# VainF/Diff-Pruning

Hardware: AMD Instinct MI355X
Metric: importance-scored images/sec (UNet fwd+bwd+|w*dL/dw|) (higher is better)
Workload: dtype f32

## Files before the change

__graft_entry__.py:

```python
import importlib
import os
import subprocess
import sys

ROOT = os.path.dirname(os.path.abspath(__file__))
PKG = os.path.join(ROOT, 'diff-pruning_amd')
SRCS = ['csrc/gemm.hip', 'csrc/norm.hip', 'csrc/elementwise.hip', 'csrc/importance.hip', 'csrc/optim.hip', 'csrc/ema.hip', 'csrc/transformer.hip', 'csrc/replay.hip', 'csrc/attention.hip', 'csrc/winograd.hip', 'csrc/winograd43.hip', 'csrc/winograd2d.hip', 'csrc/wgrad2d.hip', 'csrc/vq.hip', 'csrc/sampler.hip', 'csrc/ups9.hip', 'csrc/ldm_sampler.hip', 'csrc/evalmetrics.hip', 'csrc/prune_global.hip', 'csrc/stage.hip', 'csrc/dpm_solver.hip', 'csrc/unipc.hip', 'csrc/magnitude.hip']


def _compile(variant_flags, out_name):
    from concurrent.futures import ThreadPoolExecutor
    hipcc = '/opt/rocm/bin/hipcc' if os.path.exists('/opt/rocm/bin/hipcc') else 'hipcc'
    objdir = os.path.join(PKG, 'build', out_name)
    os.makedirs(objdir, exist_ok=True)
    common = [hipcc, '--offload-arch=gfx950', '-O3', '-std=c++17', '-fPIC', '-I' + os.path.join(ROOT, 'include')] + variant_flags
    objs = [os.path.join(objdir, os.path.basename(s_)[:-4] + '.o') for s_ in SRCS]

    def one(i):
        subprocess.check_call(common + ['-c', os.path.join(PKG, SRCS[i]), '-o', objs[i]], cwd=PKG)
    with ThreadPoolExecutor(max_workers=min(len(SRCS), os.cpu_count() or 4)) as ex:
        list(ex.map(one, range(len(SRCS))))
    subprocess.check_call([hipcc, '--offload-arch=gfx950', '-shared', '-fPIC', '-o', os.path.join(PKG, out_name)] + objs, cwd=PKG)


def build():
    _compile([], 'libdp_hip.so')
    _compile(['-DDP_IEEE_SIGMOID'], 'libdp_hip_ieee.so')
    if ROOT not in sys.path:
        sys.path.insert(0, ROOT)
    lib = importlib.import_module('diff-pruning_amd._lib')
    lib._lib = None
    handle = lib.load()
    assert handle.dp_version() >= 100
    importlib.import_module('oracle.unet_ref')
    importlib.import_module('oracle.diffusion_ref')
    importlib.import_module('oracle.pruning_ref')


def smoke():
    import time
    import torch
    t_start = time.time()
    for p in (ROOT, os.path.join(ROOT, 'tests'), os.path.join(ROOT, 'tests', 'golden')):
        if p not in sys.path:
            sys.path.insert(0, p)
    gc = importlib.import_module('diff-pruning_amd.synthetic')
    from oracle import unet_ref, diffusion_ref
    from helpers import oracle_prune_replay
    unet = importlib.import_module('diff-pruning_amd.unet')
    diffusion = importlib.import_module('diff-pruning_amd.diffusion')
    sweep = importlib.import_module('diff-pruning_amd.sweep')
    graph_mod = importlib.import_module('diff-pruning_amd.graph')
    ops = importlib.import_module('diff-pruning_amd.ops')
    assert torch.cuda.is_available(), 'smoke() needs cuda:0'
    cfg = gc.TINY_CFG
    clean = torch.from_numpy(gc.det_clean((2, 3, 16, 16), 1))
    noise = torch.from_numpy(gc.det_noise((2, 3, 16, 16), 2))

    shapes = unet_ref.param_shapes(cfg)
    P = {n: torch.from_numpy(gc.det_param(n, s, 5)).requires_grad_(True) for n, s in shapes.items()}
# ... 94 lines not shown
```

diff-pruning_amd/_lib.py:

```python
import ctypes as C
import os

_HERE = os.path.dirname(os.path.abspath(__file__))
LIB_PATH = os.environ.get('DP_HIP_LIB') or os.path.join(_HERE, 'libdp_hip.so')

c_float_p = C.c_void_p
LL = C.c_longlong


class ConvGeom(C.Structure):
    _fields_ = [(n, C.c_int) for n in ('Ho', 'Wo', 'Hs', 'Ws', 'Hv', 'Wv', 'kw', 'stride', 'sden', 'pad_t', 'pad_l',
                                       'ups', 'c_split', '_pad')] + [('x1_img_stride', LL), ('x2_img_stride', LL)]


class ConvGemmParams(C.Structure):
    _fields_ = [('A', C.c_void_p), ('a_bs', LL), ('lda', C.c_int), ('a_kc', C.c_int),
                ('X1', C.c_void_p), ('X2', C.c_void_p), ('x_bs', LL),
                ('a_bytes', C.c_uint), ('x1_bytes', C.c_uint), ('x2_bytes', C.c_uint), ('_pad0', C.c_uint),
                ('g', ConvGeom),
                ('M', C.c_int), ('C', C.c_int), ('NPIX', C.c_int), ('ntaps', C.c_int), ('batches', C.c_int),
                ('tile', C.c_int),
                ('out', C.c_void_p), ('o_img_stride', LL), ('o_bs', LL),
                ('alpha', C.c_float), ('post_scale', C.c_float),
                ('bias', C.c_void_p), ('tadd', C.c_void_p), ('tadd_stride', LL),
# ... 14 lines not shown
                ('alpha', C.c_float), ('merge', C.c_int), ('ocs', LL),
                ('o_tap_stride', LL), ('o_col_stride', C.c_int), ('xcd', C.c_int), ('col_bias', C.c_void_p)]


class AttentionParams(C.Structure):
    _fields_ = [('q', C.c_void_p), ('k', C.c_void_p), ('v', C.c_void_p), ('o', C.c_void_p),
                ('q_bs', LL), ('k_bs', LL), ('v_bs', LL), ('o_bs', LL),
                ('N', C.c_int), ('heads', C.c_int), ('d', C.c_int), ('dv', C.c_int), ('T', C.c_int), ('scale', C.c_float),
                ('variant', C.c_int), ('_pad', C.c_int)]


class Dropout(C.Structure):
    _fields_ = [('thr24', C.c_uint), ('scale', C.c_float), ('seed', C.c_ulonglong), ('site', C.c_uint), ('step', C.c_uint),
                ('n_off', LL), ('step_dev', C.c_void_p)]


class ScoreMember(C.Structure):
    _fields_ = [('w', C.c_void_p), ('g', C.c_void_p), ('R', C.c_int), ('C', C.c_int), ('T', C.c_int), ('dim', C.c_int),
                ('mode', C.c_int), ('blk0', C.c_int), ('full_off', LL), ('col_off', LL), ('idx_off', LL)]


class SliceItem(C.Structure):
    _fields_ = [('src', C.c_void_p), ('dst', C.c_void_p), ('R', C.c_int), ('C', C.c_int), ('T', C.c_int), ('dim', C.c_int),
                ('n_keep', C.c_int), ('blk0', C.c_int), ('nblk', C.c_int), ('_pad', C.c_int), ('keep_off', LL)]


class ScoreEntry(C.Structure):
    _fields_ = [('m', ScoreMember), ('score_off', LL), ('n0', C.c_int), ('_pad', C.c_int)]


class MagMember(C.Structure):
    _fields_ = [('w', C.c_void_p), ('R', C.c_int), ('C', C.c_int), ('T', C.c_int), ('dim', C.c_int), ('n0', C.c_int),
                ('blk0', C.c_int), ('fold', C.c_int), ('_pad', C.c_int), ('idx_off', LL), ('row_off', LL)]


class MagGroup(C.Structure):
    _fields_ = [('row_off', LL), ('score_off', LL), ('n0', C.c_int), ('members', C.c_int)]


class PackItem(C.Structure):
    _fields_ = [('W', C.c_void_p), ('dst', C.c_void_p), ('Co', C.c_int), ('Ci', C.c_int), ('taps', C.c_int), ('mode', C.c_int),
                ('ld', C.c_int), ('blk0', C.c_int), ('nblk', C.c_int), ('_pad', C.c_int)]


class Ups9Params(C.Structure):
    _fields_ = [('U', C.c_void_p), ('dy', C.c_void_p), ('dx', C.c_void_p), ('dy_img_stride', LL), ('dx_img_stride', LL),
                ('u_bytes', C.c_uint), ('dy_bytes', C.c_uint)] + [(n, C.c_int) for n in ('ldu', 'N', 'M', 'K', 'H', 'W',
                                                                                         'accumulate', 'tile')]


class Ups9FwdParams(C.Structure):
    _fields_ = [('U', C.c_void_p), ('x', C.c_void_p), ('bias', C.c_void_p), ('y', C.c_void_p), ('x_img_stride', LL), ('y_img_stride', LL),
                ('u_bytes', C.c_uint), ('x_bytes', C.c_uint)] + [(n, C.c_int) for n in ('ldu', 'N', 'M', 'K', 'H', 'W')]


class ColsumItem(C.Structure):
    _fields_ = [('src', C.c_void_p), ('dst', C.c_void_p), ('N', C.c_int), ('C', C.c_int), ('wstride', C.c_int),
                ('woff', C.c_int), ('accumulate', C.c_int), ('ld', C.c_int)]


class DpmSolverCoef(C.Structure):
    _fields_ = [(n, C.c_float) for n in ('sigma_s', 'alpha_s', 'kx', 'k0', 'k1', 'k2', 'ir0', 'ir1', 'q', 'iq')]


class UniPCCoef(C.Structure):
    _fields_ = [(n, C.c_float) for n in ('sigma_s', 'alpha_s', 'c_cx', 'c_c0', 'c_cB', 'c_rk1', 'c_rk2', 'c_rho1', 'c_rho2', 'c_rho_last',
                                         'p_cx', 'p_c0', 'p_cB', 'p_rk1', 'p_rk2', 'p_rho1', 'p_rho2')]


_vp, _i, _f, _ll = C.c_void_p, C.c_int, C.c_float, LL
_dr = C.POINTER(Dropout)

SIGNATURES = {
    'dp_conv_gemm': [C.POINTER(ConvGemmParams), _vp],
    'dp_conv_wino': [C.POINTER(ConvGemmParams), _vp],
    'dp_conv_wino_supported': [C.POINTER(ConvGemmParams)],
    'dp_conv_splitk_epilogue': [C.POINTER(ConvGemmParams), _vp],
    'dp_pack_weight_wino': [_vp, _i, _i, _i, _vp, _i, _vp],
    'dp_conv_wino2d': [C.POINTER(ConvGemmParams), _vp],
    'dp_conv_wino2d_supported': [C.POINTER(ConvGemmParams)],
    'dp_pack_weight_wino2d': [_vp, _i, _i, _i, _vp, _i, _vp],
    'dp_conv_wino43': [C.POINTER(ConvGemmParams), _vp],
    'dp_conv_wino43_supported': [C.POINTER(ConvGemmParams)],
    'dp_pack_weight_wino43': [_vp, _i, _i, _vp, _i, _vp],
    'dp_wgrad_wino': [C.POINTER(NtGemmParams), _vp],
    'dp_wgrad_wino2d': [C.POINTER(NtGemmParams), _vp],
    'dp_wgrad_wino2d_supported': [C.POINTER(NtGemmParams)],
    'dp_wgrad_wino_supported': [C.POINTER(NtGemmParams)],
    'dp_nt_gemm': [C.POINTER(NtGemmParams), _vp],
    'dp_splitk_reduce': [_vp, _ll, _i, _vp, _ll, _i, _vp],
    'dp_splitk_reduce_taps': [_vp, _ll, _i, _vp, _ll, _i, _i, _vp],
    'dp_pack_weight': [_vp, _i, _i, _i, _i, _vp, _i, _vp],
    'dp_pack_weight_batch': [C.POINTER(PackItem), _i, _vp],
    'dp_groupnorm_silu_fwd': [_vp, _vp, _i, _ll, _ll, _vp, _vp, _i, _i, _i, _i, _f, _i, _vp, _ll, _vp, _dr, _vp],
    'dp_groupnorm_silu_bwd': [_vp, _vp, _i, _ll, _ll, _vp, _vp, _vp, _vp, _ll, _i, _i, _i, _i, _i, _vp, _ll, _vp, _ll,
                              _vp, _ll, _vp, _dr, _vp, _vp],
    'dp_groupnorm_silu_fwd_split': [_vp, _vp, _i, _ll, _ll, _vp, _vp, _i, _i, _i, _i, _f, _i, _vp, _ll, _vp, _i, _vp, _dr,
                                    _vp],
    'dp_groupnorm_silu_bwd_split': [_vp, _vp, _i, _ll, _ll, _vp, _vp, _vp, _vp, _ll, _i, _i, _i, _i, _i, _vp, _ll, _vp, _ll,
                                    _vp, _ll, _vp, _i, _vp, _dr, _vp],
    'dp_colsum_accum': [_vp, _i, _i, _i, _i, _vp, _i, _vp],
    'dp_colsum_accum_batch': [C.POINTER(ColsumItem), _i, _vp],
    'dp_rowsum_nc': [_vp, _ll, _i, _i, _i, _vp, _vp],
    'dp_silu_fwd': [_vp, _vp, _ll, _vp],
    'dp_silu_bwd': [_vp, _vp, _vp, _ll, _i, _vp],
    'dp_axpby': [_vp, _f, _vp, _f, _ll, _vp],
    'dp_copy_strided': [_vp, _ll, _vp, _ll, _i, _ll, _i, _vp],
    'dp_attention_fwd': [C.POINTER(AttentionParams), _vp],
    'dp_attention_fwd_supported': [_i, _i, _i],
    'dp_softmax_fwd': [_vp, _vp, _ll, _i, _vp],
    'dp_softmax_bwd': [_vp, _vp, _vp, _ll, _i, _f, _vp],
    'dp_timestep_embedding': [_vp, _i, _i, _i, _f, _f, _vp, _vp],
    'dp_add_noise': [_vp, _vp, _vp, _vp, _i, _ll, _vp, _vp],
    'dp_mse_fwd_bwd': [_vp, _vp, _ll, _f, _vp, _vp, _i, _vp, _vp],
    'dp_kd_fwd_bwd': [_vp, _vp, _vp, _ll, _f, _f, _f, _vp, _vp, _i, _vp],
    'dp_kd_terms': [_vp, _i, _f, _f, _f, _vp, _vp],
    'dp_early_exit_update': [_vp, _f, _vp, _vp, _i, _vp],
    'dp_zero_if_stopped': [_vp, _ll, _vp, _vp],
    'dp_early_exit_update_ratio': [_vp, _f, _vp, _vp, _i, _vp],
    'dp_randn_philox': [_vp, _ll, _ll, C.c_ulonglong, C.c_uint, C.c_uint, _vp],
    'dp_sum_partials': [_vp, _i, _f, _vp, _vp],
    'dp_downsum2x2': [_vp, _ll, _i, _i, _i, _i, _vp, _ll, _vp],
    'dp_upsample2x': [_vp, _ll, _i, _i, _i, _i, _vp, _ll, _vp],
    'dp_interleave2x2': [_vp, _ll, _ll, _i, _i, _i, _i, _vp, _ll, _vp, _ll, _vp],
    'dp_deinterleave2x2': [_vp, _ll, _i, _i, _i, _i, _vp, _ll, _ll, _vp],
    'dp_ups_weff': [_vp, _ll, _vp, _vp],
    'dp_ups_wfold': [_vp, _ll, _vp, _i, _vp],
    'dp_ups9_u': [_vp, _ll, _vp, _vp],
    'dp_ups9_dgrad': [C.POINTER(Ups9Params), _vp],
    'dp_ups9_dgrad_supported': [C.POINTER(Ups9Params)],
    'dp_ups9_fwd': [C.POINTER(Ups9FwdParams), _vp],
    'dp_wg_reduce': [_vp, _vp, _i, _i, _i, _i, _i, _vp, _i, _vp, _vp],
    'dp_gather_add': [_vp, _vp, _i, _vp, _vp],
    'dp_group_score': [C.POINTER(ScoreMember), _i, _i, _vp, _vp, _vp, _vp],
    'dp_slice_batch': [C.POINTER(SliceItem), _i, _vp, _vp],
    'dp_score_groups': [C.POINTER(ScoreEntry), _i, _vp, _vp, _ll, _vp, _ll, _vp, _ll, _vp],
    'dp_select_smallest_workspace': [_ll, _i],
    'dp_select_smallest': [_vp, _ll, C.POINTER(LL), _i, _ll, _vp, _ll, _vp, _vp, _vp],
    'dp_magnitude_max_width': [],
    'dp_magnitude_rows': [C.POINTER(MagMember), _i, _vp, _vp, _ll, _f, _i, _vp, _ll, _vp],
    'dp_magnitude_finish': [C.POINTER(MagGroup), _i, _vp, _vp, _ll, _i, _i, _i, _vp, _ll, _vp],
    'dp_sumsq_partials': [_vp, _ll, _vp, _i, _vp],
    'dp_clip_coef': [_vp, _i, _f, _vp, _vp, _vp],
    'dp_adam_ema': [_vp, _vp, _vp, _vp, _vp, _ll, _vp, _f, _f, _f, _f, _f, _f, _f, _vp],
    'dp_set_step_scalars': [_vp, _f, _f, _f, C.c_uint, _vp],
    'dp_adamw_ema': [_vp, _vp, _vp, _vp, _vp, _ll, _vp, _f, _f, _f, _f, _f, _f, _f, _f, _vp],
    'dp_embedding_bwd': [_vp, _vp, _i, _i, _vp, _vp],
    'dp_ema_update': [_vp, _vp, _ll, _f, _vp],
    'dp_fold_sum': [_vp, C.POINTER(C.c_void_p), _i, _ll, _vp],
    'dp_adam_ema_dev': [_vp, _vp, _vp, _vp, _vp, _ll, _vp, _vp, _f, _f, _f, _f, _vp],
    'dp_ddim_step': [_vp, _vp, _vp, _f, _f, _f, _i, _f, _vp, _ll, _vp],
    'dp_ddpm_step': [_vp, _vp, _vp, _f, _f, _f, _f, _f, _i, _f, _vp, _ll, _vp],
    'dp_denoise_step': [_vp, _vp, _vp, _i, _f, _f, _f, _f, _f, _f, _vp, _vp, _ll, _vp],
    'dp_image_to_u8': [_vp, _ll, _i, _i, _i, _i, _i, _vp, _vp],
    'dp_cfg_denoise_step': [_vp, _vp, _vp, _f, _i, _vp, _vp, _vp, _f, _f, _f, _f, _f, _f, _vp, _vp, _vp, _vp, _ll, _vp],
    'dp_dpm_solver_step': [_vp, _vp, _vp, _vp, _i, _i, C.POINTER(DpmSolverCoef), _vp, _vp, _ll, _vp],
    'dp_unipc_step': [_vp, _vp, _vp, _vp, _vp, _vp, _i, _i, _i, C.POINTER(UniPCCoef), _vp, _vp, _vp, _ll, _vp],
    'dp_dropout_apply': [_vp, _ll, _vp, _ll, _i, _ll, _dr, _vp],
    'dp_dropout_mask': [_vp, _ll, _ll, _dr, _vp],
    'dp_layernorm_fwd': [_vp, _ll, _vp, _vp, _i, _i, _i, _f, _vp, _ll, _vp, _vp],
    'dp_layernorm_bwd': [_vp, _ll, _vp, _vp, _vp, _ll, _i, _i, _i, _vp, _ll, _vp, _ll, _vp, _vp],
    'dp_geglu_fwd': [_vp, _i, _ll, _vp, _vp],
    'dp_geglu_bwd': [_vp, _vp, _i, _ll, _vp, _vp],
    'dp_add_rowvec': [_vp, _ll, _vp, _i, _i, _i, _vp, _ll, _vp],
    'dp_q_sample': [_vp, _vp, _vp, _vp, _vp, _i, _ll, _vp, _vp],
    'dp_cfg_combine': [_vp, _vp, _f, _vp, _ll, _vp],
    'dp_u8_to_float': [_vp, _i, _i, _i, _i, _i, _vp, _ll, _i, C.c_uint, _i, _dr, _vp],
    'dp_pool2d': [_vp, _ll, _i, _i, _i, _i, _i, _i, _i, _i, _vp, _ll, _vp],
    'dp_resize_bilinear': [_vp, _ll, _i, _i, _i, _i, _i, _i, _f, _f, _vp, _vp],
    'dp_ssim': [_vp, _vp, _i, _i, _i, _i, _f, _vp, _vp, _vp],
    'dp_ssim_workspace': [_i, _i, _i, _i],
    'dp_mse_per_image': [_vp, _vp, _i, _ll, _vp, _vp],
    'dp_em_row_norms2': [_vp, _ll, _i, _ll, _vp, _vp],
    'dp_em_knn_merge': [_vp, _ll, _ll, _ll, _vp, _vp, _i, _i, _vp, _vp],
    'dp_em_inside_ball': [_vp, _ll, _ll, _ll, _vp, _vp, _vp, _vp, _vp],
    'dp_em_poly_sums': [_vp, _i, _ll, _ll, _ll, _ll, C.c_double, C.c_double, _i, _vp, _i, _vp, _vp],
    'dp_em_isc_rows': [_vp, _ll, _i, _ll, _vp, _vp, _vp],
    'dp_em_isc_colmeans': [_vp, _ll, _vp, _ll, _ll, _i, _vp, _vp],
    'dp_vq_blocks': [_ll],
    'dp_vq_quantize': [_vp, _ll, _i, _i, _ll, _vp, _i, _vp, _ll, _vp, _vp, _vp],
    'dp_vq_loss': [_vp, _i, C.c_double, _vp, _vp],
    'dp_replay_build': [_vp, C.POINTER(C.c_void_p)],
    'dp_replay_launch': [_vp, _vp, _vp],
    'dp_replay_info': [_vp, C.POINTER(C.c_int)],
# ... 35 lines not shown
```

diff-pruning_amd/engine.py:

```python
import os

import torch

from . import ops

_SPEC3 = ops.ConvSpec(3, 1, 1, 0)
_SPEC1 = ops.ConvSpec(1, 1, 0, 0)
_SPEC_UP = ops.ConvSpec(3, 1, 1, 1)
UPS_COPY = not os.environ.get('DP_NO_UPS_COPY')
UPS_SUBPIXEL = not os.environ.get('DP_NO_UPS_SUBPIXEL')
_UPS_SPECS = ops.UPS_CLASS_SPECS
S2_PARITY = not os.environ.get('DP_NO_S2_PARITY')
FUSE_QKV_WGRAD = not os.environ.get('DP_NO_FUSED_QKV_WGRAD')
OVERLAP_MIN_WORK = 4_000_000

RES_DIFFUSERS = dict(norm1='.norm1', conv1='.conv1', temb='.time_emb_proj', norm2='.norm2', conv2='.conv2',
                     shortcut='.conv_shortcut', dropout='.dropout')
RES_LDM = dict(norm1='.in_layers.0', conv1='.in_layers.2', temb='.emb_layers.1', norm2='.out_layers.0',
               conv2='.out_layers.3', shortcut='.skip_connection')


SIDE_KEEP_MAX_BYTES = int(float(os.environ.get('DP_SIDE_KEEP_GB', '4')) * (1 << 30))


# ... 375 lines not shown
                  alpha=1.0, dx_add=None):
        w = self.P[name + '.weight']

        if rows is None and (name + '.bias') in self.P and self._rows_src is not None and self._rows_src[0].data_ptr() == dy.data_ptr():
            rows = self._rows_of(dy)

        def param_grads(rows):
            ops.conv_wgrad(dy, x, x2, self.G[name + '.weight'], spec, alpha=alpha, accumulate=True)
            if (name + '.bias') in self.P:
                if rows is None:
                    rows = ops.rowsum_nc(dy)
                if alpha != 1.0:
                    rows = rows.contiguous()
                    rows = ops.axpby(rows, alpha, torch.empty_like(rows), 0.0)
                self._colsum(rows, rows.shape[0], rows.shape[1], 1, 0, self.G[name + '.bias'])

        side = self._side_stream(dy, x, x2, rows)
        if side is None:
            param_grads(rows)
        else:
            with torch.cuda.stream(side):
                param_grads(rows)
        if not need_dx:
            return None
        if (S2_PARITY and spec.stride == 2 and spec.k == 3 and not spec.ups and spec.pad in (0, 1) and alpha == 1.0
                and dx_out is None and in_hw[0] == 2 * dy.shape[2] and in_hw[1] == 2 * dy.shape[3]):
            packs = [self.packs.get(name, w, ('s2', ph, pw, spec.pad)) for ph in (0, 1) for pw in (0, 1)]
            return ops.conv_dgrad_s2(dy, packs, w.shape[1], spec, in_hw, add=dx_add)
        wd, ldd = self.packs.get(name, w, 1)
        wino = None
        if w.dim() == 4 and w.shape[2] == 3 and hasattr(ops, 'wino_wanted') and tuple(in_hw) == tuple(dy.shape[2:]):
            wino = self._wino_operand(name, w, 1, w.shape[1], (w.shape[0],), dy.shape[0], dy.shape[2], dy.shape[3], spec)
        dx = ops.conv_dgrad(dy, wd, ldd, w.shape[1], spec, in_hw, alpha=alpha, out=dx_out, accumulate=dx_accumulate,
                            **({'wino': wino} if wino is not None else {}))
        if dx_add is not None:
            ops.copy_strided(dx_add, dx, accumulate=True)
        return dx

    def _ups_conv_fwd(self, name, x):
        w = self.P[name + '.weight']
        N, _, H, W = x.shape
        if hasattr(ops, 'ups9_fwd_wanted') and ops.ups9_fwd_wanted(N, w.shape[1], w.shape[0], H, W):
            up, ldu = self.packs.get(name, w, ('up9', 0, 0))
            return ops.ups9_fwd(x, up, ldu, w.shape[0], bias=self.P.get(name + '.bias'))
        q = ops.empty_act((4, N, w.shape[0], H, W), x.device)
        for c, spec in enumerate(_UPS_SPECS):
            wp, ld = self.packs.get(name, w, ('up', c, 0))
            ops.conv_forward(x, None, wp, ld, w.shape[0], spec, bias=self.P.get(name + '.bias'), out=q[c])
        return ops.interleave2x2(q)

    def _ups_conv_bwd(self, name, dy, x):
        w = self.P[name + '.weight']
        use9 = hasattr(ops, 'ups9_dgrad_wanted') and ops.ups9_dgrad_wanted(x.shape[0], w.shape[1], w.shape[0], x.shape[2], x.shape[3])
        dyq = None if use9 else ops.deinterleave2x2(dy)
        rows = None
        if (name + '.bias') in self.P and self._rows_src is not None and self._rows_src[0].data_ptr() == dy.data_ptr():
            rows = self._rows_of(dy)

        def param_grads(rows, dyq=dyq):
            if dyq is None:
                dyq = ops.deinterleave2x2(dy)
            gweff = torch.empty((4,) + tuple(w.shape[:2]) + (2, 2), dtype=torch.float32, device=dy.device)
            for c, spec in enumerate(_UPS_SPECS):
                ops.conv_wgrad(dyq[c], x, None, gweff[c], spec, accumulate=False)
            ops.ups_wfold(gweff, self.G[name + '.weight'], accumulate=True)
            if (name + '.bias') in self.P:
                if rows is None:
                    rows = ops.rowsum_nc(dy)
                self._colsum(rows, rows.shape[0], rows.shape[1], 1, 0, self.G[name + '.bias'])

        side = self._side_stream(dy, dyq, x, rows)
        if side is None:
            param_grads(rows)
        else:
            with torch.cuda.stream(side):
                param_grads(rows)
        if use9:
            up, ldu = self.packs.get(name, w, ('up9', 0, 1))
            return ops.ups9_dgrad(dy, up, ldu, w.shape[1])
        dx = None
        for c, spec in enumerate(_UPS_SPECS):
            wd, ldd = self.packs.get(name, w, ('up', c, 1))
            dx = ops.conv_dgrad(dyq[c], wd, ldd, w.shape[1], spec, tuple(x.shape[2:]), out=dx, accumulate=c > 0)
        return dx

    def _gn_param_grads(self, name, pws):
        N, C = pws.shape[0], pws.shape[1]
        self._colsum(pws, N, C, 2, 1, self.G[name + '.weight'])
        self._colsum(pws, N, C, 2, 0, self.G[name + '.bias'])

    def resnet_fwd(self, pre, xa, xb, semb, out_scale, save, names=RES_DIFFUSERS, G=None, eps=None):
        P, cfg = self.P, self.cfg
        G = cfg['norm_num_groups'] if G is None else G
        eps = cfg['norm_eps'] if eps is None else eps
        nm = names
        n1, st1 = ops.groupnorm_fwd(xa, xb, P[pre + nm['norm1'] + '.weight'], P[pre + nm['norm1'] + '.bias'], G, eps, True)
        if self._temb is not None:
            o, c = self._temb[1][pre]
            tproj = self._temb[2][:xa.shape[0], o:o + c]
        elif semb is None:
            tproj = None
        else:
            tproj = self._linear(pre + nm['temb'], semb)
        h = self._conv(pre + nm['conv1'], n1, None, _SPEC3, tadd=tproj)
        drop = self._drop(pre + nm['dropout']) if 'dropout' in nm else None
        n2, st2 = ops.groupnorm_fwd(h, None, P[pre + nm['norm2'] + '.weight'], P[pre + nm['norm2'] + '.bias'], G, eps, True,
                                    drop=drop)
        has_sc = (pre + nm['shortcut'] + '.weight') in P
        if has_sc:
            res = self._conv(pre + nm['shortcut'], xa, xb, _SPEC1)
        else:
            if xb is not None:
                res = torch.cat([xa, xb], 1)
            else:
                res = xa
        out = self._conv(pre + nm['conv2'], n2, None, _SPEC3, res=res, post_scale=1.0 / out_scale)
        if save is not None:
            save[pre] = (xa, xb, st1, n1, h, st2, n2, has_sc, out_scale, nm, G, drop)
# ... 315 lines not shown
```

diff-pruning_amd/ops.py:

```python
import ctypes as C
import os
import math
import torch

from . import _lib as L

_f32 = torch.float32


def _lib():
    return L.load()


_raw_stream = getattr(torch._C, '_cuda_getCurrentRawStream', None)


def _stream():
    if _raw_stream is not None:
        return C.c_void_p(_raw_stream(torch.cuda.current_device()))
    return C.c_void_p(torch.cuda.current_stream().cuda_stream)


def _p(t):
    return None if t is None else C.c_void_p(t.data_ptr())
# ... 709 lines not shown
    HW = H * W
    npix = HW * N
    if npix >= (1 << 29):
        return False
    if 9 * Cin * ldu * 4 != u_bytes or u_bytes >= _MAX_BYTES:
        return False
    if x_img_stride < HW * Cin or y_img_stride < 4 * HW * Cout or (y_img_stride & 1):
        return False
    if x_bytes < ((N - 1) * x_img_stride + HW * Cin) * 4 or x_bytes >= _MAX_BYTES:
        return False
    bm, bn = UPS9_FWD_TILE
    return -(-npix // bn) * -(-Cout // bm) < (1 << 31)


def ups9_fwd_gate(N, Cin, Cout, H, W):
    bm, bn = UPS9_FWD_TILE
    blocks = -(-(N * H * W) // bn) * -(-Cout // bm)
    return blocks >= UPS9_FWD_GATE_MIN_BLOCKS and max(Cin, Cout) <= UPS9_FWD_GATE_MAX_CH


def ups9_fwd_wanted(N, Cin, Cout, H, W):
    if not UPS9 or min(N, Cin, Cout, H, W) < 1 or N * H * W * max(Cin, 4 * Cout) * 4 >= _MAX_BYTES:
        return False
    return ups9_fwd_gate(N, Cin, Cout, H, W)


def _ups9_fwd_params(x, up, ldu, Cout, bias, out):
    sx, so = _chk_act(x), _chk_act(out)
    N, Cin, H, W = x.shape
    p = L.Ups9FwdParams()
    p.U, p.x, p.bias, p.y = _p(up), _p(x), _p(bias), _p(out)
    p.x_img_stride, p.y_img_stride = sx, so
    p.u_bytes, p.x_bytes = up.numel() * 4, _extent_bytes(x)
    p.ldu, p.N, p.M, p.K, p.H, p.W = ldu, N, Cout, Cin, H, W
    return p


def ups9_fwd(x, up, ldu, Cout, *, bias=None, out=None):
    N, Cin, H, W = x.shape
    if out is None:
        out = empty_act((N, Cout, 2 * H, 2 * W), x.device)
    assert out.shape == (N, Cout, 2 * H, 2 * W) and (bias is None or (bias.numel() == Cout and bias.is_contiguous()))
    p = _ups9_fwd_params(x, up, ldu, Cout, bias, out)
    ok = ups9_fwd_shape_ok(N, Cin, Cout, H, W, p.x_img_stride, p.y_img_stride, p.x_bytes, ldu, p.u_bytes, up.data_ptr(),
                           out.data_ptr(), bias.data_ptr() if bias is not None else 0)
    if not ok:
        raise ValueError('dp_ups9_fwd does not take this launch (ups9_fwd_shape_ok)')
    rc = _run(lambda: _lib().dp_ups9_fwd(C.byref(p), _stream()),
              _UPS9_FWD_NAME,
              2.0 * Cin * N * H * W * Cout * 9, 4.0 * (x.numel() + up.numel() + out.numel()))
    assert rc != 1, 'host shape rule and dp_ups9_fwd disagree (hipErrorInvalidValue for a launch ups9_fwd_shape_ok takes)'
    L.check(rc, 'dp_ups9_fwd')
    return out


_ws_cache = {}
WGRAD_BLOCKS = 1024
WGRAD_MIN_PIX = int(os.environ.get('DP_WGRAD_MIN_PIX', '128'))


def _workspace(n, device):
    if torch.cuda.is_current_stream_capturing():
        return torch.empty(max(n, 1), dtype=_f32, device=device)
    key = (device.index if device.index is not None else torch.cuda.current_device(), _stream().value)
    t = _ws_cache.get(key)
    if t is None or t.numel() < n:
        t = torch.empty(max(n, 1 << 22), dtype=_f32, device=device)
        _ws_cache[key] = t
    return t


WGRAD_WINO = os.environ.get('DP_WGRAD_WINO', '1') not in ('0', '')
WGRAD_WINO_MIN_FILL = float(os.environ.get('DP_WGRAD_WINO_MIN_FILL', '0.7'))
WGRAD_WINO_MIN_WORK = int(os.environ.get('DP_WGRAD_WINO_MIN_WORK', '512'))


WGRAD_WINO2D = os.environ.get('DP_WGRAD_WINO2D', '1') not in ('0', '')
WGRAD_WINO2D_BLOCKS = int(os.environ.get('DP_WGRAD_WINO2D_BLOCKS', '512'))
WGRAD_WINO2D_MIN_FILL = float(os.environ.get('DP_WGRAD_WINO2D_MIN_FILL', '0.7'))


def _nt_gemm_params(A, a_img_stride, x, x2, geom, M, Cc, ncols, ntaps, P, splits, pps, tile, alpha, ldo, batch=None):
    p = L.NtGemmParams()
    Z, a_bs, x_bs, batched = batch or (1, 0, 0, 0)
    p.A, p.a_bs, p.a_img_stride = _p(A), a_bs, a_img_stride
    p.X1, p.X2, p.x_bs = _p(x), _p(x2), x_bs
    if batch is None:
        p.a_bytes, p.x1_bytes, p.x2_bytes = _extent_bytes(A), _extent_bytes(x), _extent_bytes(x2)
    else:
        p.a_bytes, p.x1_bytes, p.x2_bytes = _checked_bytes(M * P * 4), _checked_bytes(ncols * P * 4), 0
    p.g = geom
    p.M, p.C, p.NCOLS, p.ntaps, p.P = M, Cc, ncols, ntaps, P
    p.batches, p.splits, p.p_per_split, p.tile, p.batched = Z, splits, pps, tile, batched
    p.alpha, p.ldo = alpha, ldo
    return p


def _wgrad_launch(p, gw, accumulate, sym, name, flops, label, taps, device):
    acc = 1 if accumulate else 0
    if p.splits == 1:
        p.out, p.o_bs, p.accumulate = _p(gw), 0, acc
        L.check(_run(lambda: getattr(_lib(), sym)(C.byref(p), _stream()), name, flops), label)
        return gw
    n = gw.numel()
    ws = _workspace(p.splits * n, device)
    p.out, p.o_bs, p.accumulate = _p(ws), n, 0
# ... 1069 lines not shown
```

include/dp_hip.h:

```cpp
#ifndef DP_HIP_H
#define DP_HIP_H
#include <stdint.h>
#ifdef __cplusplus
extern "C" {
#endif

typedef struct dp_conv_geom {
    int Ho, Wo, Hs, Ws, Hv, Wv, kw, stride, sden, pad_t, pad_l, ups, c_split, _pad;
    long long x1_img_stride, x2_img_stride;
} dp_conv_geom;

typedef struct dp_conv_gemm_params {
    const float* A; long long a_bs; int lda; int a_kc;
    const float* X1; const float* X2; long long x_bs;
    unsigned a_bytes, x1_bytes, x2_bytes, _pad0;
    dp_conv_geom g;
    int M, C, NPIX, ntaps, batches, tile;
    float* out; long long o_img_stride; long long o_bs;
    float alpha; float post_scale;
    const float* bias; const float* tadd; long long tadd_stride;
    const float* res; long long r_img_stride;
    int accumulate; int ksplit;
    float* ws;
    int x_guard; int act;
// ... 94 lines not shown
    long long q_bs, k_bs, v_bs, o_bs;
    int N, heads, d, dv, T;
    float scale;
    int variant;
    int _pad;
} dp_attention_params;
int dp_attention_fwd(const dp_attention_params* p, void* stream);
int dp_attention_fwd_supported(int T, int d, int dv);
int dp_softmax_bwd(const float* p, const float* dp, float* ds, long long rows, int cols, float scale, void* stream);

int dp_timestep_embedding(const float* t, int B, int dim, int flip_sin_to_cos, float freq_shift, float max_period, float* out, void* stream);

int dp_add_noise(const float* x0, const float* noise, const float* acp, const int64_t* t, int B, long long per_img, float* out, void* stream);

int dp_mse_fwd_bwd(const float* out, const float* noise, long long n, float gscale, float* dout, float* partial, int nblocks,
                   const float* stop_state, void* stream);
int dp_kd_fwd_bwd(const float* out, const float* teacher, const float* noise, long long n, float w_kd, float w_eps, float gscale,
                  float* dout, float* partial, int nblocks, void* stream);
int dp_kd_terms(const float* partial, int nblocks, float w_kd, float w_eps, float scale, float* terms, void* stream);
int dp_early_exit_update(const float* loss, float thr, float* state, float* losses, int max_steps, void* stream);
int dp_zero_if_stopped(float* x, long long n, const float* state, void* stream);
int dp_early_exit_update_ratio(const float* loss, float thr, float* state, float* losses, int max_steps, void* stream);
int dp_sum_partials(const float* partial, int n, float scale, float* dst, void* stream);

int dp_downsum2x2(const float* dy, long long dy_img_stride, int N, int C, int H, int W, float* dx, long long dx_img_stride, void* stream);

int dp_upsample2x(const float* x, long long x_img_stride, int N, int C, int H, int W, float* y, long long y_img_stride, void* stream);

int dp_interleave2x2(const float* q, long long q_class_stride, long long q_img_stride, int N, int C, int Ho, int Wo,
                     const float* add, long long add_img_stride, float* dx, long long dx_img_stride, void* stream);

int dp_deinterleave2x2(const float* y, long long y_img_stride, int N, int C, int Ho, int Wo, float* q,
                       long long q_class_stride, long long q_img_stride, void* stream);

int dp_ups_weff(const float* w, long long M, float* weff, void* stream);
int dp_ups_wfold(const float* gweff, long long M, float* gw, int accumulate, void* stream);

typedef struct dp_ups9_params {
    const float* U; const float* dy; float* dx;
    long long dy_img_stride, dx_img_stride;
    unsigned u_bytes, dy_bytes;
    int ldu, N, M, K, H, W, accumulate, tile;
} dp_ups9_params;
int dp_ups9_u(const float* w, long long M, float* u, void* stream);
int dp_ups9_dgrad(const dp_ups9_params* p, void* stream);
int dp_ups9_dgrad_supported(const dp_ups9_params* p);
typedef struct dp_ups9_fwd_params {
    const float* U; const float* x; const float* bias; float* y;
    long long x_img_stride, y_img_stride;
    unsigned u_bytes, x_bytes;
    int ldu, N, M, K, H, W;
} dp_ups9_fwd_params;
int dp_ups9_fwd(const dp_ups9_fwd_params* p, void* stream);

int dp_wg_reduce(const float* w, const float* g, int R, int C, int T, int dim, int mode, float* out, int accumulate,
                 float* scratch, void* stream);

int dp_gather_add(const float* src, const int64_t* idx, int n, float* dst, void* stream);

typedef struct dp_score_member {
    const float* w; const float* g;
    int R, C, T, dim, mode, blk0;
    long long full_off, col_off, idx_off;
} dp_score_member;
int dp_group_score(const dp_score_member* members, int n, int n0, const int64_t* idx, float* scratch, float* score, void* stream);
typedef struct dp_slice_item {
    const float* src; float* dst;
    int R, C, T, dim, n_keep, blk0, nblk, _pad;
    long long keep_off;
} dp_slice_item;
int dp_slice_batch(const dp_slice_item* items, int n, const int64_t* keep, void* stream);

typedef struct dp_score_entry {
    dp_score_member m;
    long long score_off;
    int n0, _pad;
} dp_score_entry;
int dp_score_groups(dp_score_entry* entries, int n, dp_score_entry* table_dev, const int64_t* idx, long long idx_len,
                    float* scratch, long long scratch_len, float* scores, long long n_scores, void* stream);
long long dp_select_smallest_workspace(long long n, int groups);
int dp_select_smallest(const float* scores, long long n, const long long* group_off, int groups, long long k, void* work,
                       long long work_bytes, int* out_dev, int* out_host, void* stream);

typedef struct dp_mag_member {
    const float* w;
    int R, C, T, dim, n0, blk0, fold, _pad;
    long long idx_off, row_off;
} dp_mag_member;
typedef struct dp_mag_group {
    long long row_off, score_off;
    int n0, members;
} dp_mag_group;
int dp_magnitude_max_width(void);
int dp_magnitude_rows(dp_mag_member* members, int n, dp_mag_member* table_dev, const int64_t* idx, long long idx_len,
                      float p, int root, float* rows, long long rows_len, void* stream);
int dp_magnitude_finish(const dp_mag_group* groups, int n, dp_mag_group* table_dev, const float* rows, long long rows_len,
                        int reduction, int normalizer, int lamp, float* scores, long long n_scores, void* stream);

int dp_sumsq_partials(const float* x, long long n, float* partial, int nblocks, void* stream);
int dp_set_step_scalars(float* hyper, float lr, float bc1, float bc2, unsigned step, void* stream);
int dp_adam_ema_dev(float* p, const float* g, float* m, float* v, float* ema, long long n, const float* clip_coef,
                    const float* hyper, float b1, float b2, float eps, float ema_decay, void* stream);
int dp_clip_coef(const float* partial, int n, float max_norm, float* norm_out, float* coef_out, void* stream);
int dp_adam_ema(float* p, const float* g, float* m, float* v, float* ema, long long n, const float* clip_coef,
                float lr, float b1, float b2, float eps, float bc1, float bc2, float ema_decay, void* stream);

// ... 106 lines not shown
```

Baseline: 5054.

## Add fused upsample-conv weight-gradient kernel with split-K MFMA and reduce

Adds a dedicated kernel for the weight gradient of the nearest-2x upsample followed by a 3x3 conv. It reads the interleaved dy directly and forms nine combined dy/x tap panels in shared memory, so one MFMA GEMM covers every tap. A split-K reduce kernel then folds the result back into 3x3 weights. This replaces deinterleaving dy, four separate conv_wgrad launches and the ups_wfold pass for large enough shapes. The trade-offs are a workspace of splits*9*Co*Ci floats and an extra reduce pass.

```diff
diff --git a/__graft_entry__.py b/__graft_entry__.py
--- a/__graft_entry__.py
+++ b/__graft_entry__.py
@@ -5,7 +5,7 @@
 
 ROOT = os.path.dirname(os.path.abspath(__file__))
 PKG = os.path.join(ROOT, 'diff-pruning_amd')
-SRCS = ['csrc/gemm.hip', 'csrc/norm.hip', 'csrc/elementwise.hip', 'csrc/importance.hip', 'csrc/optim.hip', 'csrc/ema.hip', 'csrc/transformer.hip', 'csrc/replay.hip', 'csrc/attention.hip', 'csrc/winograd.hip', 'csrc/winograd43.hip', 'csrc/winograd2d.hip', 'csrc/wgrad2d.hip', 'csrc/vq.hip', 'csrc/sampler.hip', 'csrc/ups9.hip', 'csrc/ldm_sampler.hip', 'csrc/evalmetrics.hip', 'csrc/prune_global.hip', 'csrc/stage.hip', 'csrc/dpm_solver.hip', 'csrc/unipc.hip', 'csrc/magnitude.hip']
+SRCS = ['csrc/gemm.hip', 'csrc/norm.hip', 'csrc/elementwise.hip', 'csrc/importance.hip', 'csrc/optim.hip', 'csrc/ema.hip', 'csrc/transformer.hip', 'csrc/replay.hip', 'csrc/attention.hip', 'csrc/winograd.hip', 'csrc/winograd43.hip', 'csrc/winograd2d.hip', 'csrc/wgrad2d.hip', 'csrc/vq.hip', 'csrc/sampler.hip', 'csrc/ups9.hip', 'csrc/ups9_wgrad.hip', 'csrc/ldm_sampler.hip', 'csrc/evalmetrics.hip', 'csrc/prune_global.hip', 'csrc/stage.hip', 'csrc/dpm_solver.hip', 'csrc/unipc.hip', 'csrc/magnitude.hip']
 
 
 def _compile(variant_flags, out_name):
diff --git a/diff-pruning_amd/_lib.py b/diff-pruning_amd/_lib.py
--- a/diff-pruning_amd/_lib.py
+++ b/diff-pruning_amd/_lib.py
@@ -90,6 +90,12 @@
 class Ups9FwdParams(C.Structure):
     _fields_ = [('U', C.c_void_p), ('x', C.c_void_p), ('bias', C.c_void_p), ('y', C.c_void_p), ('x_img_stride', LL), ('y_img_stride', LL),
                 ('u_bytes', C.c_uint), ('x_bytes', C.c_uint)] + [(n, C.c_int) for n in ('ldu', 'N', 'M', 'K', 'H', 'W')]
+
+
+class Ups9WgradParams(C.Structure):
+    _fields_ = [('dy', C.c_void_p), ('x', C.c_void_p), ('ws', C.c_void_p), ('gw', C.c_void_p), ('dy_img_stride', LL), ('x_img_stride', LL),
+                ('ws_floats', LL), ('dy_bytes', C.c_uint), ('x_bytes', C.c_uint)] + [(n, C.c_int) for n in (
+                    'N', 'Co', 'Ci', 'H', 'W', 'splits', 'tiles_per_split', 'ld', 'accumulate')]
 
 
 class ColsumItem(C.Structure):
@@ -168,6 +174,8 @@
     'dp_ups9_dgrad': [C.POINTER(Ups9Params), _vp],
     'dp_ups9_dgrad_supported': [C.POINTER(Ups9Params)],
     'dp_ups9_fwd': [C.POINTER(Ups9FwdParams), _vp],
+    'dp_ups9_wgrad': [C.POINTER(Ups9WgradParams), _vp],
+    'dp_ups9_wgrad_reduce': [C.POINTER(Ups9WgradParams), _vp],
     'dp_wg_reduce': [_vp, _vp, _i, _i, _i, _i, _i, _vp, _i, _vp, _vp],
     'dp_gather_add': [_vp, _vp, _i, _vp, _vp],
     'dp_group_score': [C.POINTER(ScoreMember), _i, _i, _vp, _vp, _vp, _vp],
diff --git a/diff-pruning_amd/csrc/ups9_wgrad.hip b/diff-pruning_amd/csrc/ups9_wgrad.hip
--- /dev/null
+++ b/diff-pruning_amd/csrc/ups9_wgrad.hip
@@ -0,0 +1,246 @@
+#include "dp_common.h"
+
+#define U9W_LAUNCH(k, ...) do { dp_launch_names[dp_launches++ & (DP_LAUNCH_RING - 1)] = #k; hipLaunchKernelGGL(k, __VA_ARGS__); } while (0)
+
+typedef float f32x2 __attribute__((ext_vector_type(2)));
+
+#define U9W_RSRC_FLAGS 0x00020000
+#define U9W_OOB 0x80000000u
+#define U9W_BM 64
+#define U9W_BN 64
+#define U9W_KP 16
+#define U9W_LD 66
+
+__device__ __forceinline__ __amdgpu_buffer_rsrc_t u9w_rsrc(const float* base, unsigned bytes) {
+    return __builtin_amdgcn_make_buffer_rsrc((void*)base, 0, (int)bytes, U9W_RSRC_FLAGS);
+}
+__device__ __forceinline__ float u9w_bload(__amdgpu_buffer_rsrc_t r, unsigned byte_off) {
+    asm volatile("" : "+v"(byte_off));
+    return __builtin_bit_cast(float, __builtin_amdgcn_raw_buffer_load_b32(r, (int)byte_off, 0, 0));
+}
+__device__ __forceinline__ f32x2 u9w_bload2(__amdgpu_buffer_rsrc_t r, unsigned byte_off) {
+    asm volatile("" : "+v"(byte_off));
+    return __builtin_bit_cast(f32x2, __builtin_amdgcn_raw_buffer_load_b64(r, (int)byte_off, 0, 0));
+}
+
+__global__ __launch_bounds__(256, 2) void ups9_wgrad_kernel(const dp_ups9_wgrad_params p) {
+    constexpr int BM = U9W_BM, BN = U9W_BN, KP = U9W_KP, LD = U9W_LD;
+    constexpr int PT = BM * KP / 256;
+    constexpr int NS = 9 * KP / 2;
+    static_assert(BM == 64 && BN == 64 && KP == 16 && PT == 4 && LD >= BM && LD >= BN, "tile");
+    __shared__ __attribute__((aligned(16))) float Ds[9 * KP * LD];
+    __shared__ __attribute__((aligned(16))) float Vs[9 * KP * LD];
+
+    const int tid = threadIdx.x;
+    const int lane = tid & 63;
+    const int wave = __builtin_amdgcn_readfirstlane(tid >> 6);
+    const int li = lane & 31, lk = lane >> 5;
+    const int wm0 = (wave >> 1) * 32, wn0 = (wave & 1) * 32;
+    const int H = p.H, W = p.W, HW = H * W, W2 = 2 * W, HW4 = 4 * HW;
+    const int Co = p.Co, Ci = p.Ci;
+    const int NPIX = p.N * HW;
+    const int NKT = (NPIX + KP - 1) / KP;
+    const int CT = (Ci + BN - 1) / BN;
+    const int TILES = ((Co + BM - 1) / BM) * CT;
+    int tile, split;
+    {
+        const int b = blockIdx.x;
+        if (!(p.splits & 7)) {
+            const int xcd = b & 7, slot = b >> 3;
+            tile = slot % TILES;
+            split = (slot / TILES) * 8 + xcd;
+        } else {
+            tile = b % TILES;
+            split = b / TILES;
+        }
+    }
+    const int m0 = (tile / CT) * BM, c0 = (tile % CT) * BN;
+    const int kt0 = split * p.tiles_per_split;
+    const int kt1 = kt0 + p.tiles_per_split < NKT ? kt0 + p.tiles_per_split : NKT;
+
+    const int ppix = tid & 15, pch = 4 * wave + ((lane >> 4) & 3);
+    const __amdgpu_buffer_rsrc_t rD = u9w_rsrc(p.dy, p.dy_bytes);
+    const __amdgpu_buffer_rsrc_t rX = u9w_rsrc(p.x, p.x_bytes);
+
+    f32x2 dr[PT][2];
+    float xr[PT][9];
+    auto load_tile = [&](int kt) {
+        const int pixel = kt * KP + ppix;
+        const bool pvalid = pixel < NPIX;
+        const int n = pixel / HW, rem = pixel - n * HW;
+        const int i = rem / W, j = rem - i * W;
+        const int dbase = (int)(n * p.dy_img_stride) + (2 * i) * W2 + 2 * j;
+        const int xbase = (int)(n * p.x_img_stride) + (i - 1) * W + (j - 1);
+        const bool top = i > 0, bot = i < H - 1, left = j > 0, right = j < W - 1;
+#pragma unroll
+        for (int q = 0; q < PT; ++q) {
+            const int co = m0 + pch + 16 * q;
+            const bool ok = pvalid && co < Co;
+            const int off = dbase + co * HW4;
+            dr[q][0] = u9w_bload2(rD, ok ? (unsigned)(off * 4) : U9W_OOB);
+            dr[q][1] = u9w_bload2(rD, ok ? (unsigned)((off + W2) * 4) : U9W_OOB);
+        }
+#pragma unroll
+        for (int q = 0; q < PT; ++q) {
+            const int ci = c0 + pch + 16 * q;
+            const bool ok = pvalid && ci < Ci;
+            const int off0 = xbase + ci * HW;
+#pragma unroll
+            for (int r = 0; r < 3; ++r) {
+                const bool rok = ok && (r == 0 ? top : r == 2 ? bot : true);
+#pragma unroll
+                for (int c = 0; c < 3; ++c) {
+                    const bool v = rok && (c == 0 ? left : c == 2 ? right : true);
+                    xr[q][3 * r + c] = u9w_bload(rX, v ? (unsigned)((off0 + r * W + c) * 4) : U9W_OOB);
+                }
+            }
+        }
+    };
+    auto store_tile = [&]() {
+#pragma unroll
+        for (int q = 0; q < PT; ++q) {
+            const float d00 = dr[q][0][0], d01 = dr[q][0][1], d10 = dr[q][1][0], d11 = dr[q][1][1];
+            const float r0 = d00 + d01, r2 = d10 + d11;
+            float* o = &Ds[ppix * LD + pch + 16 * q];
+            o[0 * KP * LD] = d00;
+            o[1 * KP * LD] = r0;
+            o[2 * KP * LD] = d01;
+            o[3 * KP * LD] = d00 + d10;
+            o[4 * KP * LD] = r0 + r2;
+            o[5 * KP * LD] = d01 + d11;
+            o[6 * KP * LD] = d10;
+            o[7 * KP * LD] = r2;
+            o[8 * KP * LD] = d11;
+        }
+#pragma unroll
+        for (int q = 0; q < PT; ++q) {
+            const float* d = xr[q];
+            float t[3][3];
+#pragma unroll
+            for (int c = 0; c < 3; ++c) {
+                t[0][c] = d[c] - d[3 + c];
+                t[1][c] = d[3 + c];
+                t[2][c] = d[6 + c] - d[3 + c];
+            }
+            float* o = &Vs[ppix * LD + pch + 16 * q];
+#pragma unroll
+            for (int a = 0; a < 3; ++a) {
+                o[(3 * a + 0) * KP * LD] = t[a][0] - t[a][1];
+                o[(3 * a + 1) * KP * LD] = t[a][1];
+                o[(3 * a + 2) * KP * LD] = t[a][2] - t[a][1];
+            }
+        }
+    };
+
+    f32x16 acc[9];
+#pragma unroll
+    for (int t = 0; t < 9; ++t)
+#pragma unroll
+        for (int r = 0; r < 16; ++r) acc[t][r] = 0.f;
+
+    if (kt0 < kt1) load_tile(kt0);
+    for (int kt = kt0; kt < kt1; ++kt) {
+        __syncthreads();
+        store_tile();
+        __syncthreads();
+        if (kt + 1 < kt1) load_tile(kt + 1);
+        float a[3], b[3];
+        auto frag = [&](int s, float& fa, float& fb) {
+            const int kk = (s % 9) * KP + (s / 9) * 2 + lk;
+            fa = Ds[kk * LD + wm0 + li];
+            fb = Vs[kk * LD + wn0 + li];
+        };
+        frag(0, a[0], b[0]);
+        frag(1, a[1], b[1]);
+#pragma unroll
+        for (int s = 0; s < NS; ++s) {
+            if (s + 2 < NS) frag(s + 2, a[(s + 2) % 3], b[(s + 2) % 3]);
+            __builtin_amdgcn_sched_barrier(0);
+            acc[s % 9] = __builtin_amdgcn_mfma_f32_32x32x2f32(a[s % 3], b[s % 3], acc[s % 9], 0, 0, 0);
+            __builtin_amdgcn_sched_barrier(0);
+        }
+    }
+
+    const int col = c0 + wn0 + li;
+    if (col >= Ci) return;
+#pragma unroll
+    for (int t = 0; t < 9; ++t) {
+        float* o = p.ws + ((long long)split * 9 + t) * Co * (long long)p.ld + col;
+#pragma unroll
+        for (int r = 0; r < 16; ++r) {
+            const int row = m0 + wm0 + (r & 3) + 8 * (r >> 2) + 4 * lk;
+            if (row < Co) o[(long long)row * p.ld] = acc[t][r];
+        }
+    }
+}
+
+__global__ __launch_bounds__(256) void ups9_wgrad_reduce_kernel(const float* __restrict__ ws, int splits, int Co, int Ci, int ld,
+                                                                float* __restrict__ gw, int accumulate) {
+    const int idx = blockIdx.x * 256 + threadIdx.x;
+    if (idx >= Co * Ci) return;
+    const int co = idx / Ci, ci = idx - co * Ci;
+    const long long tap_stride = (long long)Co * ld, split_stride = 9 * tap_stride;
+    const float* s = ws + (long long)co * ld + ci;
+    float u[3][3];
+#pragma unroll
+    for (int t = 0; t < 9; ++t) u[t / 3][t % 3] = s[t * tap_stride];
+    for (int z = 1; z < splits; ++z) {
+        s += split_stride;
+#pragma unroll
+        for (int t = 0; t < 9; ++t) u[t / 3][t % 3] += s[t * tap_stride];
+    }
+    float g[3][3];
+#pragma unroll
+    for (int b = 0; b < 3; ++b) {
+        g[0][b] = u[0][b] + u[1][b];
+        g[1][b] = u[1][b];
+        g[2][b] = u[1][b] + u[2][b];
+    }
+    float* o = gw + (long long)idx * 9;
+#pragma unroll
+    for (int r = 0; r < 3; ++r) {
+        const float v0 = g[r][0] + g[r][1], v1 = g[r][1], v2 = g[r][1] + g[r][2];
+        o[3 * r + 0] = accumulate ? o[3 * r + 0] + v0 : v0;
+        o[3 * r + 1] = accumulate ? o[3 * r + 1] + v1 : v1;
+        o[3 * r + 2] = accumulate ? o[3 * r + 2] + v2 : v2;
+    }
+}
+
+static int dp_ups9_wgrad_supported(const dp_ups9_wgrad_params* pp) {
+    if (!pp) return 0;
+    const dp_ups9_wgrad_params& p = *pp;
+    if (!p.dy || !p.x || !p.ws || !p.gw) return 0;
+    if (((uintptr_t)p.dy & 7) || ((uintptr_t)p.x & 3) || ((uintptr_t)p.ws & 3) || ((uintptr_t)p.gw & 3)) return 0;
+    if (p.N < 1 || p.Co < 1 || p.Ci < 1 || p.H < 1 || p.W < 1 || p.splits < 1 || p.tiles_per_split < 1) return 0;
+    if (p.ld < p.Ci || p.ws_floats < (long long)p.splits * 9 * p.Co * p.ld) return 0;
+    const long long HW = (long long)p.H * p.W;
+    const long long npix = HW * p.N;
+    if (npix >= (1ll << 29)) return 0;
+    if (p.dy_img_stride < 4 * HW * p.Co || (p.dy_img_stride & 1) || p.x_img_stride < HW * p.Ci) return 0;
+    const long long dy_need = ((p.N - 1) * p.dy_img_stride + 4 * HW * p.Co) * 4;
+    const long long x_need = ((p.N - 1) * p.x_img_stride + HW * p.Ci) * 4;
+    if ((long long)p.dy_bytes < dy_need || p.dy_bytes >= 0x80000000u) return 0;
+    if ((long long)p.x_bytes < x_need || p.x_bytes >= 0x80000000u) return 0;
+    const long long nkt = (npix + U9W_KP - 1) / U9W_KP;
+    if ((long long)p.splits * p.tiles_per_split < nkt || (long long)(p.splits - 1) * p.tiles_per_split >= nkt) return 0;
+    const long long tiles = (long long)((p.Co + U9W_BM - 1) / U9W_BM) * ((p.Ci + U9W_BN - 1) / U9W_BN);
+    if (tiles * p.splits >= (1ll << 31) || (long long)p.Co * p.Ci >= (1ll << 31)) return 0;
+    return 1;
+}
+
+extern "C" int dp_ups9_wgrad(const dp_ups9_wgrad_params* pp, void* stream) {
+    if (!dp_ups9_wgrad_supported(pp)) return (int)hipErrorInvalidValue;
+    const dp_ups9_wgrad_params& p = *pp;
+    const long long tiles = (long long)((p.Co + U9W_BM - 1) / U9W_BM) * ((p.Ci + U9W_BN - 1) / U9W_BN);
+    U9W_LAUNCH(ups9_wgrad_kernel, dim3((unsigned)(tiles * p.splits)), dim3(256), 0, (hipStream_t)stream, p);
+    return DP_LAUNCH_CHECK();
+}
+
+extern "C" int dp_ups9_wgrad_reduce(const dp_ups9_wgrad_params* pp, void* stream) {
+    if (!dp_ups9_wgrad_supported(pp)) return (int)hipErrorInvalidValue;
+    const dp_ups9_wgrad_params& p = *pp;
+    const unsigned nb = (unsigned)(((long long)p.Co * p.Ci + 255) / 256);
+    U9W_LAUNCH(ups9_wgrad_reduce_kernel, dim3(nb), dim3(256), 0, (hipStream_t)stream, (const float*)p.ws, p.splits, p.Co, p.Ci, p.ld, p.gw,
+               p.accumulate);
+    return DP_LAUNCH_CHECK();
+}
diff --git a/diff-pruning_amd/engine.py b/diff-pruning_amd/engine.py
--- a/diff-pruning_amd/engine.py
+++ b/diff-pruning_amd/engine.py
@@ -451,18 +451,22 @@
     def _ups_conv_bwd(self, name, dy, x):
         w = self.P[name + '.weight']
         use9 = hasattr(ops, 'ups9_dgrad_wanted') and ops.ups9_dgrad_wanted(x.shape[0], w.shape[1], w.shape[0], x.shape[2], x.shape[3])
+        wg9 = hasattr(ops, 'ups9_wgrad_wanted') and ops.ups9_wgrad_wanted(x.shape[0], w.shape[1], w.shape[0], x.shape[2], x.shape[3])
         dyq = None if use9 else ops.deinterleave2x2(dy)
         rows = None
         if (name + '.bias') in self.P and self._rows_src is not None and self._rows_src[0].data_ptr() == dy.data_ptr():
             rows = self._rows_of(dy)
 
         def param_grads(rows, dyq=dyq):
-            if dyq is None:
-                dyq = ops.deinterleave2x2(dy)
-            gweff = torch.empty((4,) + tuple(w.shape[:2]) + (2, 2), dtype=torch.float32, device=dy.device)
-            for c, spec in enumerate(_UPS_SPECS):
-                ops.conv_wgrad(dyq[c], x, None, gweff[c], spec, accumulate=False)
-            ops.ups_wfold(gweff, self.G[name + '.weight'], accumulate=True)
+            if wg9:
+                ops.ups9_wgrad(dy, x, self.G[name + '.weight'])
+            else:
+                if dyq is None:
+                    dyq = ops.deinterleave2x2(dy)
+                gweff = torch.empty((4,) + tuple(w.shape[:2]) + (2, 2), dtype=torch.float32, device=dy.device)
+                for c, spec in enumerate(_UPS_SPECS):
+                    ops.conv_wgrad(dyq[c], x, None, gweff[c], spec, accumulate=False)
+                ops.ups_wfold(gweff, self.G[name + '.weight'], accumulate=True)
             if (name + '.bias') in self.P:
                 if rows is None:
                     rows = ops.rowsum_nc(dy)
diff --git a/diff-pruning_amd/ops.py b/diff-pruning_amd/ops.py
--- a/diff-pruning_amd/ops.py
+++ b/diff-pruning_amd/ops.py
@@ -785,6 +785,87 @@
     assert rc != 1, 'host shape rule and dp_ups9_fwd disagree (hipErrorInvalidValue for a launch ups9_fwd_shape_ok takes)'
     L.check(rc, 'dp_ups9_fwd')
     return out
+
+
+UPS9_WGRAD = os.environ.get('DP_UPS9_WGRAD', '1') not in ('0', '')
+UPS9_WGRAD_TILE = (64, 64, 16)
+_UPS9_WGRAD_NAMES = ('ups9_wgrad_kernel', 'ups9_wgrad_reduce_kernel')
+UPS9_WGRAD_BLOCKS = 512
+UPS9_WGRAD_GATE_MIN_PIX, UPS9_WGRAD_GATE_MIN_CH = 256, 128
+
+
+def ups9_wgrad_splits(N, Cin, Cout, H, W, splits=None):
+    bm, bn, kp = UPS9_WGRAD_TILE
+    tiles = -(-Cout // bm) * -(-Cin // bn)
+    nkt = -(-(N * H * W) // kp)
+    if splits is None:
+        splits = min(UPS9_WGRAD_BLOCKS // tiles, nkt // 4)
+    splits = max(1, min(splits, nkt))
+    tps = -(-nkt // splits)
+    return -(-nkt // tps), tps
+
+
+def ups9_wgrad_shape_ok(N, Cin, Cout, H, W, dy_img_stride, x_img_stride, dy_bytes, x_bytes, ld, splits, tiles_per_split, ws_floats,
+                        dy_ptr=0, x_ptr=0, ws_ptr=0, gw_ptr=0):
+    if (dy_ptr & 7) or (x_ptr & 3) or (ws_ptr & 3) or (gw_ptr & 3):
+        return False
+    if min(N, Cin, Cout, H, W, splits, tiles_per_split) < 1:
+        return False
+    if ld < Cin or ws_floats < splits * 9 * Cout * ld:
+        return False
+    HW = H * W
+    npix = HW * N
+    if npix >= (1 << 29):
+        return False
+    if dy_img_stride < 4 * HW * Cout or (dy_img_stride & 1) or x_img_stride < HW * Cin:
+        return False
+    if dy_bytes < ((N - 1) * dy_img_stride + 4 * HW * Cout) * 4 or dy_bytes >= _MAX_BYTES:
+        return False
+    if x_bytes < ((N - 1) * x_img_stride + HW * Cin) * 4 or x_bytes >= _MAX_BYTES:
+        return False
+    bm, bn, kp = UPS9_WGRAD_TILE
+    nkt = -(-npix // kp)
+    if splits * tiles_per_split < nkt or (splits - 1) * tiles_per_split >= nkt:
+        return False
+    return -(-Cout // bm) * -(-Cin // bn) * splits < (1 << 31) and Cout * Cin < (1 << 31)
+
+
+def ups9_wgrad_gate(N, Cin, Cout, H, W):
+    return N * H * W >= UPS9_WGRAD_GATE_MIN_PIX and min(Cin, Cout) >= UPS9_WGRAD_GATE_MIN_CH
+
+
+def ups9_wgrad_wanted(N, Cin, Cout, H, W):
+    if not UPS9 or not UPS9_WGRAD or min(N, Cin, Cout, H, W) < 1 or N * H * W * max(Cin, 4 * Cout) * 4 >= _MAX_BYTES:
+        return False
+    return ups9_wgrad_gate(N, Cin, Cout, H, W)
+
+
+def ups9_wgrad(dy, x, gw, *, accumulate=True, splits=None):
+    sd, sx = _chk_act(dy), _chk_act(x)
+    N, Cout, H2, W2 = dy.shape
+    _, Cin, H, W = x.shape
+    assert x.shape[0] == N and H2 == 2 * H and W2 == 2 * W
+    assert gw.shape == (Cout, Cin, 3, 3) and gw.is_contiguous() and gw.dtype == _f32
+    splits, tps = ups9_wgrad_splits(N, Cin, Cout, H, W, splits)
+    n = splits * 9 * Cout * Cin
+    ws = _workspace(n, dy.device)
+    p = L.Ups9WgradParams()
+    p.dy, p.x, p.ws, p.gw = _p(dy), _p(x), _p(ws), _p(gw)
+    p.dy_img_stride, p.x_img_stride, p.ws_floats = sd, sx, ws.numel()
+    p.dy_bytes, p.x_bytes = _extent_bytes(dy), _extent_bytes(x)
+    p.N, p.Co, p.Ci, p.H, p.W = N, Cout, Cin, H, W
+    p.splits, p.tiles_per_split, p.ld, p.accumulate = splits, tps, Cin, 1 if accumulate else 0
+    ok = ups9_wgrad_shape_ok(N, Cin, Cout, H, W, sd, sx, p.dy_bytes, p.x_bytes, p.ld, splits, tps, p.ws_floats, dy.data_ptr(),
+                             x.data_ptr(), ws.data_ptr(), gw.data_ptr())
+    if not ok:
+        raise ValueError('dp_ups9_wgrad does not take this launch (ups9_wgrad_shape_ok)')
+    rc = _run(lambda: _lib().dp_ups9_wgrad(C.byref(p), _stream()), _UPS9_WGRAD_NAMES[0], 18.0 * Cout * Cin * N * H * W,
+              4.0 * (dy.numel() + x.numel() + n))
+    assert rc != 1, 'host shape rule and dp_ups9_wgrad disagree (hipErrorInvalidValue for a launch ups9_wgrad_shape_ok takes)'
+    L.check(rc, 'dp_ups9_wgrad')
+    L.check(_run(lambda: _lib().dp_ups9_wgrad_reduce(C.byref(p), _stream()), _UPS9_WGRAD_NAMES[1], 0.0, 4.0 * (n + gw.numel())),
+            'dp_ups9_wgrad_reduce')
+    return gw
 
 
 _ws_cache = {}
diff --git a/include/dp_hip.h b/include/dp_hip.h
--- a/include/dp_hip.h
+++ b/include/dp_hip.h
@@ -170,6 +170,14 @@
     int ldu, N, M, K, H, W;
 } dp_ups9_fwd_params;
 int dp_ups9_fwd(const dp_ups9_fwd_params* p, void* stream);
+typedef struct dp_ups9_wgrad_params {
+    const float* dy; const float* x; float* ws; float* gw;
+    long long dy_img_stride, x_img_stride, ws_floats;
+    unsigned dy_bytes, x_bytes;
+    int N, Co, Ci, H, W, splits, tiles_per_split, ld, accumulate;
+} dp_ups9_wgrad_params;
+int dp_ups9_wgrad(const dp_ups9_wgrad_params* p, void* stream);
+int dp_ups9_wgrad_reduce(const dp_ups9_wgrad_params* p, void* stream);
 
 int dp_wg_reduce(const float* w, const float* g, int R, int C, int T, int dim, int mode, float* out, int accumulate,
                  float* scratch, void* stream);
```

Result: faster. 5112, median of 6 (+1.2%).
